# microsoft/ANCE

Hardware: NVIDIA H100
Metric: ANN-refresh throughput: passages encoded/sec + queries top-200/sec, 8.8M x 768 (higher is better)
Workload: dtype fp16

## Files before the change

### ance_b200/csrc/capi.cu

```cuda
#include <atomic>
#include <mutex>
#include <string.h>
#include <vector>

#include "common.h"
#include "gemm_store.cuh"

namespace ance {

static thread_local char g_err[1024] = "";
std::atomic<int64_t> g_launches{0};

void set_error(const char* fmt, ...) {
  va_list ap;
  va_start(ap, fmt);
  vsnprintf(g_err, sizeof(g_err), fmt, ap);
  va_end(ap);
}

void count_launch(int n) { g_launches.fetch_add(n, std::memory_order_relaxed); }

static bool g_prof_on = false;
static std::mutex g_prof_mu;
static std::vector<cudaEvent_t> g_ev_pool;
// ... 9 lines not shown
}
void prof_begin(int cls, cudaStream_t st) {
  if (!g_prof_on) return;
  std::lock_guard<std::mutex> lk(g_prof_mu);
  g_open[cls] = get_event();
  cudaEventRecord(g_open[cls], st);
}
void prof_end(int cls, cudaStream_t st) {
  if (!g_prof_on) return;
  std::lock_guard<std::mutex> lk(g_prof_mu);
  cudaEvent_t b = get_event();
  cudaEventRecord(b, st);
  g_spans[cls].push_back({g_open[cls], b});
}

}

extern "C" const char* ance_version(void) { return "ance_b200 0.1 (sm_90a)"; }
extern "C" const char* ance_last_error(void) { return ance::g_err; }
extern "C" int64_t ance_launch_count(void) { return ance::g_launches.load(); }

extern "C" int ance_profile_enable(int on) {
  std::lock_guard<std::mutex> lk(ance::g_prof_mu);
  ance::g_prof_on = on != 0;
  return ANCE_OK;
}

extern "C" int ance_profile_read(double* ms_by_class, int64_t* launches_by_class, int n, int reset) {
  ANCE_REQUIRE(ms_by_class && launches_by_class && n > 0 && n <= ance::kNumCls, "ance_profile_read: bad arguments");
  ANCE_CUDA(cudaDeviceSynchronize());
  std::lock_guard<std::mutex> lk(ance::g_prof_mu);
  for (int c = 0; c < ance::kNumCls; ++c) {
    for (auto& s : ance::g_spans[c]) {
      float ms = 0.f;
      if (cudaEventElapsedTime(&ms, s.a, s.b) == cudaSuccess) { ance::g_ms[c] += ms; ance::g_cnt[c] += 1; }
      ance::g_ev_pool.push_back(s.a);
      ance::g_ev_pool.push_back(s.b);
    }
    ance::g_spans[c].clear();
  }
  for (int c = 0; c < n; ++c) { ms_by_class[c] = ance::g_ms[c]; launches_by_class[c] = ance::g_cnt[c]; }
  if (reset) for (int c = 0; c < ance::kNumCls; ++c) { ance::g_ms[c] = 0; ance::g_cnt[c] = 0; }
  return ANCE_OK;
}

namespace {

template <int BN, int STAGES, int CG, uint32_t FMT>
int run_dbg(const void* A, const void* B, int M, int N, int K, const float* bias, const void* R, int act, void* C,
            float* C32, cudaStream_t st) {
  constexpr int EW = 4;
  using Ep = gemm::EpStore<BN, EW>;
  CUtensorMap tmA, tmB;
  if (!tc05_host::make_tmap_2d_16b(&tmA, A, M, K, K, gemm::BM) ||
      !tc05_host::make_tmap_2d_16b(&tmB, B, N, K, K, BN / CG)) {
    ance::set_error("cuTensorMapEncodeTiled failed (M=%d N=%d K=%d)", M, N, K);
    return ANCE_ERR_CUDA;
  }
  gemm::WorkShape ws = gemm::make_shape(M, N, K, BN, CG, 0);
  typename Ep::Params p;
  memset(&p, 0, sizeof(p));
  if (C && !gemm::make_store_tmap(&p.tmC, C, M, N, N)) {
    ance::set_error("cuTensorMapEncodeTiled failed for the output (M=%d N=%d)", M, N);
    return ANCE_ERR_CUDA;
  }
  if (C && R && !gemm::make_store_tmap(&p.tmR, const_cast<void*>(R), M, N, N)) {
    ance::set_error("cuTensorMapEncodeTiled failed for the residual (M=%d N=%d)", M, N);
    return ANCE_ERR_CUDA;
  }
  p.C = reinterpret_cast<uint16_t*>(C);
  p.C32 = C32;
  p.bias = bias;
  p.R = reinterpret_cast<const uint16_t*>(R);
  p.ldc = N;
  p.ldc32 = N;
  p.ldr = N;
  p.act = act;
  ANCE_CUDA((gemm::launch<Ep, BN, STAGES, CG, EW, FMT>(tmA, tmB, ws, p, 0, st)));
  ance::count_launch(1);
  return ANCE_OK;
}

template <uint32_t FMT>
int dispatch_dbg(int variant, const void* A, const void* B, int M, int N, int K, const float* bias, const void* R,
                 int act, void* C, float* C32, cudaStream_t st) {
  switch (variant) {
    case 0: return run_dbg<128, 4, 1, FMT>(A, B, M, N, K, bias, R, act, C, C32, st);
    case 1: return run_dbg<128, 3, 1, FMT>(A, B, M, N, K, bias, R, act, C, C32, st);
    case 2: return run_dbg<128, 4, 2, FMT>(A, B, M, N, K, bias, R, act, C, C32, st);
    case 3: return run_dbg<64, 6, 2, FMT>(A, B, M, N, K, bias, R, act, C, C32, st);
    case 4: return run_dbg<64, 6, 1, FMT>(A, B, M, N, K, bias, R, act, C, C32, st);
    default: ance::set_error("ance_dbg_gemm: unknown variant %d", variant); return ANCE_ERR_INVALID;
  }
}

}

extern "C" int ance_dbg_gemm(const void* A_dev, const void* B_dev, int M, int N, int K, int fmt, int variant,
                             const float* bias_dev, const void* residual_bf16_dev, int act, void* C_bf16_dev,
                             float* C_f32_dev, void* stream) {
  ANCE_REQUIRE(A_dev && B_dev && M > 0 && N > 0 && K > 0, "ance_dbg_gemm: null operand or empty shape");
  ANCE_REQUIRE(K % 8 == 0 && N % 8 == 0, "ance_dbg_gemm: K and N must be multiples of 8 (16-byte rows)");
  cudaStream_t st = reinterpret_cast<cudaStream_t>(stream);
  if (fmt == ANCE_FMT_BF16)
    return dispatch_dbg<tc05::kFmtBF16>(variant, A_dev, B_dev, M, N, K, bias_dev, residual_bf16_dev, act, C_bf16_dev,
                                        C_f32_dev, st);
  if (fmt == ANCE_FMT_FP16)
    return dispatch_dbg<tc05::kFmtF16>(variant, A_dev, B_dev, M, N, K, bias_dev, residual_bf16_dev, act, C_bf16_dev,
                                       C_f32_dev, st);
  ance::set_error("ance_dbg_gemm: unknown operand format %d", fmt);
  return ANCE_ERR_INVALID;
}
```

### ance_b200/csrc/encoder.cu

```cuda
#include <math.h>
#include <stdlib.h>
#include <string.h>

#include <cmath>
#include <map>
#include <vector>

#include "attention.cuh"
#include "attn_bwd_long.cuh"
#include "common.h"
#include "dropout.cuh"
#include "encoder_bwd.cuh"
#include "gemm_store.cuh"

namespace {

constexpr float kLog2e = 1.4426950408889634f;

struct EmbedParams {
  const int32_t* ids;
  const int32_t* lens;
  const uint8_t* mask;
  int B, L, H;
  int roberta;
// ... 375 lines not shown
  float *word = nullptr, *pos = nullptr, *type = nullptr;
  float *eg = nullptr, *eb = nullptr;
  std::vector<LayerDev> layers;
  uint16_t* head_w = nullptr;
  float *head_b = nullptr, *head_g = nullptr, *head_bt = nullptr;
  uint16_t *X = nullptr, *QKV = nullptr, *CTX = nullptr, *T = nullptr, *X1 = nullptr, *FF = nullptr;
  float* kbias = nullptr;
  uint16_t *cls_ctx = nullptr, *cls_x = nullptr;
  int32_t* seq_row0 = nullptr;
  int32_t *row_lo = nullptr, *row_hi = nullptr;
  int2* tile_kv = nullptr;
  float* head_tmp = nullptr;
  int* err_flag = nullptr;
  uint16_t* dbg = nullptr;
  int dbg_tokens = 0;
  float* dbg_grads = nullptr;
  int dbg_grads_tokens = 0;
  bool dbg_grads_valid = false;
  int prune_last_layer = 1;
  int varlen_align = 1;
  std::vector<void*> allocs;
  struct TrainRecord {
    int B, L;
    float p_hidden, p_attn;
    uint64_t seed;
    int n_tiles;
  };
  std::map<const void*, TrainRecord> train_shapes;
  int train_max_len = 128;
  struct LayerT { uint16_t *wqkv, *wo, *w1, *w2; };
  std::vector<LayerT> wt;
  uint16_t* head_wt = nullptr;
  bool wt_stale = true;
  void* bwd_scratch = nullptr;
  std::vector<bwd::RefreshPiece> refresh_table;
  bwd::RefreshPiece* refresh_dev = nullptr;
  size_t refresh_cap = 0;
  size_t bwd_scratch_bytes = 0;
};

namespace {

int require_sm90(int* dev_out) {
  int dev = 0, major = 0, minor = 0;
  ANCE_CUDA(cudaGetDevice(&dev));
  cudaDeviceGetAttribute(&major, cudaDevAttrComputeCapabilityMajor, dev);
  cudaDeviceGetAttribute(&minor, cudaDevAttrComputeCapabilityMinor, dev);
  if (major != 9 || minor != 0) {
    ance::set_error("device %d has compute capability %d.%d; libance_b200 is built for sm_90a only (no CPU fallback)", dev, major, minor);
    return ANCE_ERR_CUDA;
  }
  if (dev_out) *dev_out = dev;
  return ANCE_OK;
}

template <class T>
T* dev_alloc(ance_encoder* e, size_t n) {
  void* p = nullptr;
  if (cudaMalloc(&p, n * sizeof(T)) != cudaSuccess) return nullptr;
  e->allocs.push_back(p);
  return reinterpret_cast<T*>(p);
}

float* upload_f32(ance_encoder* e, const float* h, size_t n) {
  float* d = dev_alloc<float>(e, n);
  if (d) cudaMemcpy(d, h, n * 4, cudaMemcpyHostToDevice);
  return d;
}

uint16_t* upload_16(ance_encoder* e, const float* h, size_t n) {
  std::vector<uint16_t> tmp(n);
  if (e->fmt == tc05::kFmtBF16) for (size_t i = 0; i < n; ++i) tmp[i] = act16::Act<tc05::kFmtBF16>::from_float_host(h[i]);
  else for (size_t i = 0; i < n; ++i) tmp[i] = act16::Act<tc05::kFmtF16>::from_float_host(h[i]);
  uint16_t* d = dev_alloc<uint16_t>(e, n);
  if (d) cudaMemcpy(d, tmp.data(), n * 2, cudaMemcpyHostToDevice);
  return d;
}

int gelu_form() {
  static const int form = getenv("ANCE_B200_GELU") ? atoi(getenv("ANCE_B200_GELU")) : 2;
  return form;
}

template <uint32_t FMT, bool kDrop = false>
int linear(const uint16_t* A, size_t lda, int M, const uint16_t* W, int N, int K, const float* bias,
           const uint16_t* R, int act, uint16_t* C, float* C32, cudaStream_t st, int cls = ance::kClsGemm,
           size_t ldr = 0, const drop::Cfg* dc = nullptr) {
  constexpr int BN = 128, CG = 1, EW = 4, STAGES = 4;
  using Ep = gemm::EpStore<BN, EW, FMT, kDrop>;
  CUtensorMap tmA, tmB;
  if (!tc05_host::make_tmap_2d_16b(&tmA, A, M, K, lda, gemm::BM) || !tc05_host::make_tmap_2d_16b(&tmB, W, N, K, K, BN / CG)) {
    ance::set_error("encoder: cuTensorMapEncodeTiled failed (M=%d N=%d K=%d)", M, N, K);
    return ANCE_ERR_CUDA;
  }
  gemm::WorkShape ws = gemm::make_shape(M, N, K, BN, CG, 0);
  typename Ep::Params p;
  memset(&p, 0, sizeof(p));
  if (C && !gemm::make_store_tmap(&p.tmC, C, M, N, N)) {
    ance::set_error("encoder: cuTensorMapEncodeTiled failed for the output (M=%d N=%d)", M, N);
    return ANCE_ERR_CUDA;
  }
  if (ldr == 0) ldr = N;
  if (C && R && !gemm::make_store_tmap(&p.tmR, const_cast<uint16_t*>(R), M, N, static_cast<int>(ldr))) {
    ance::set_error("encoder: cuTensorMapEncodeTiled failed for the residual (M=%d N=%d)", M, N);
    return ANCE_ERR_CUDA;
  }
  p.C = C;
  p.C32 = C32;
  p.bias = bias;
  p.R = R;
  p.ldc = N;
  p.ldc32 = N;
  p.ldr = static_cast<int>(ldr);
  p.act = act;
  if constexpr (kDrop) p.drop = *dc;
  {
    ance::ProfScope ps(cls, st);
    ANCE_CUDA((gemm::launch<Ep, BN, STAGES, CG, EW, FMT>(tmA, tmB, ws, p, 0, st)));
  }
  ance::count_launch(1);
  return ANCE_OK;
}

int g_ln_rows_per_warp = 2;

template <uint32_t FMT>
int layer_norm(const void* in, bool in_f32, size_t in_ld, int rows, int H, const float* g, const float* b, float eps,
               uint16_t* out16, float* out32, cudaStream_t st) {
  const int blocks = (rows + 7) / 8;
  const int nv = H / 256;
  ance::ProfScope ps(ance::kClsNorm, st);
  if (!in_f32 && out16 && !out32 && nv == 3 && g_ln_rows_per_warp > 1 && rows >= 4096) {
    const uint16_t* src = reinterpret_cast<const uint16_t*>(in);
    if (g_ln_rows_per_warp == 2) ln_rows_multi_kernel<3, 2, FMT><<<(rows + 15) / 16, 256, 0, st>>>(src, in_ld, rows, H, g, b, eps, out16);
    else if (g_ln_rows_per_warp == 3) ln_rows_packed_kernel<3, 2, FMT><<<(rows + 15) / 16, 256, 0, st>>>(src, in_ld, rows, H, g, b, eps, out16);
    else ln_rows_multi_kernel<3, 4, FMT><<<(rows + 31) / 32, 256, 0, st>>>(src, in_ld, rows, H, g, b, eps, out16);
    ANCE_CUDA(cudaGetLastError());
    ance::count_launch(1);
    return ANCE_OK;
  }
#define LN_CASE(NV_)                                                                                            \
  if (in_f32) ln_rows_kernel<NV_, true, FMT><<<blocks, 256, 0, st>>>(in, in_ld, rows, H, g, b, eps, out16, out32); \
  else ln_rows_kernel<NV_, false, FMT><<<blocks, 256, 0, st>>>(in, in_ld, rows, H, g, b, eps, out16, out32)
  if (nv == 3) { LN_CASE(3); }
  else if (nv == 4) { LN_CASE(4); }
  else if (nv == 1) { LN_CASE(1); }
  else if (nv == 2) { LN_CASE(2); }
  else { ance::set_error("encoder: hidden size %d unsupported", H); return ANCE_ERR_UNSUPPORTED; }
#undef LN_CASE
  ANCE_CUDA(cudaGetLastError());
  ance::count_launch(1);
  return ANCE_OK;
}

template <uint32_t FMT>
int set_attention_attrs() {
  ANCE_CUDA(cudaFuncSetAttribute(attn::attention_multi_kernel<false, FMT>, cudaFuncAttributeMaxDynamicSharedMemorySize, attn::Smem::kDynamic));
  ANCE_CUDA(cudaFuncSetAttribute(attn::attention_single_kernel<false, FMT>, cudaFuncAttributeMaxDynamicSharedMemorySize, attn::SmemSingle::kDynamic));
  ANCE_CUDA(cudaFuncSetAttribute(attn::attention_single_kernel<true, FMT>, cudaFuncAttributeMaxDynamicSharedMemorySize, attn::SmemSingle::kDynamic));
  ANCE_CUDA(cudaFuncSetAttribute(attn::attention_multi_kernel<true, FMT>, cudaFuncAttributeMaxDynamicSharedMemorySize, attn::Smem::kDynamic));
  ANCE_CUDA(cudaFuncSetAttribute(attn::attention_single_kernel<false, FMT, true>, cudaFuncAttributeMaxDynamicSharedMemorySize, attn::SmemSingle::kDynamic));
  ANCE_CUDA(cudaFuncSetAttribute(attn::attention_single_kernel<true, FMT, true>, cudaFuncAttributeMaxDynamicSharedMemorySize, attn::SmemSingle::kDynamic));
  ANCE_CUDA(cudaFuncSetAttribute(attn::attention_multi_kernel<false, FMT, true>, cudaFuncAttributeMaxDynamicSharedMemorySize, attn::Smem::kDynamic));
  ANCE_CUDA(cudaFuncSetAttribute(attn::attention_multi_kernel<true, FMT, true>, cudaFuncAttributeMaxDynamicSharedMemorySize, attn::Smem::kDynamic));
  return ANCE_OK;
}

struct AttentionLaunch {
  CUtensorMap tmQKV, tmCTX;
  attn::Params ap;
  int grid;
  bool packed, single;
};

int make_attention(AttentionLaunch& a, const uint16_t* qkv, uint16_t* ctx, int n_tokens, int L, int heads,
                   const float* kbias, const int32_t* row_lo, const int32_t* row_hi, const int2* tile_kv) {
  const int H = heads * attn::kDh;
  if (!tc05_host::make_tmap_2d_16b(&a.tmQKV, qkv, n_tokens, 3 * H, 3 * H, attn::kTile)) {
    ance::set_error("encoder: cuTensorMapEncodeTiled failed for QKV");
    return ANCE_ERR_CUDA;
  }
  if (!tc05_host::make_tmap_2d_16b(&a.tmCTX, ctx, n_tokens, H, H, attn::kTile)) {
    ance::set_error("encoder: cuTensorMapEncodeTiled failed for the attention output");
    return ANCE_ERR_CUDA;
  }
// ... 1561 lines not shown
```

### ance_b200/csrc/gemm_core.cuh

```cuda
#pragma once
#include "tc05.cuh"

namespace gemm {

using namespace tc05;

constexpr int BM = 128;
constexpr int BK = 64;
constexpr int MMA_K = 16;

struct WorkShape {
  int M, N, K;
  int num_m_blks;
  int num_n_blks;
  int n_splits;
  int n_blks_per_split;
  unsigned long long hint_a, hint_b;
  int* pace;
  int pace_window;
  int pace_stride;
};

static __device__ __noinline__ void pace_wait(int* pace, int window, int me, int n_clusters, int stride, int seq) {
  volatile int* vp = pace;
// ... 110 lines not shown
  } else if (warp >= 4 && warp < 8) {
    Ring<STAGES> ring;
    uint32_t acc_phase = 0;
    auto release = [&](int stage) {
      __syncwarp();
      if (lane == 0) {
        mbar_arrive(&empty_bar[stage]);
        if constexpr (CG == 2) mbar_arrive_cluster(&empty_bar[stage], cta_rank ^ 1u);
      }
    };
    for (int w = cluster_id; w < total_work; w += num_clusters) {
      const int m_blk = w / ws.n_splits, split = w - m_blk * ws.n_splits;
      const int nb0 = split * ws.n_blks_per_split;
      const int nb1 = min(nb0 + ws.n_blks_per_split, ws.num_n_blks);
      (void)m_blk;
      for (int nb = nb0; nb < nb1; ++nb) {
        float acc0[BN / 2], acc1[BN / 2];
#pragma unroll
        for (int i = 0; i < BN / 2; ++i) acc0[i] = acc1[i] = 0.f;
        int prev_stage = -1;
        for (int kb = 0; kb < num_kb; ++kb) {
          mbar_wait(&full_bar[ring.stage], ring.phase, 3);
          const uint32_t sa = smem_u32(smem + ring.stage * Plan::kStageBytes);
          const uint32_t sb = sa + Plan::kABytes;
          wgmma_fence();
#pragma unroll
          for (int k = 0; k < BK / MMA_K; ++k) {
            const uint64_t bdesc = make_desc_k_sw128(sb + k * MMA_K * 2);
            wgmma_tile<FMT, BN>(acc0, make_desc_k_sw128(sa + k * MMA_K * 2), bdesc, 1u);
            wgmma_tile<FMT, BN>(acc1, make_desc_k_sw128(sa + 64 * 128 + k * MMA_K * 2), bdesc, 1u);
          }
          wgmma_commit();
          wgmma_wait<1>();
          wgmma_fence_regs(acc0);
          wgmma_fence_regs(acc1);
          if (prev_stage >= 0) release(prev_stage);
          prev_stage = ring.stage;
          ring.advance();
        }
        wgmma_wait<0>();
        wgmma_fence_regs(acc0);
        wgmma_fence_regs(acc1);
        if (prev_stage >= 0) release(prev_stage);
        mbar_wait(aempty_bar, acc_phase ^ 1, 2);
        acc_store_frag(acc_tile, Plan::kAccPitch, 0, 0, acc0);
        acc_store_frag(acc_tile, Plan::kAccPitch, 64, 0, acc1);
        __syncwarp();
        if (lane == 0) mbar_arrive(afull_bar);
        acc_phase ^= 1;
      }
    }
  } else if (warp >= 8) {
    Ep epi;
    EpiCtx cx;
    cx.quad = warp & 3;
    cx.epi_warp = warp - 8;
    cx.lane = lane;
    cx.work_seq = 0;
    cx.ep_smem = smem + Plan::kEpOffset;
    uint32_t acc_phase = 0;
    const uint32_t tacc = smem_u32(acc_tile) / 4u + static_cast<uint32_t>((cx.quad * 32 + lane) * Plan::kAccPitch);
    for (int w = cluster_id; w < total_work; w += num_clusters, ++cx.work_seq) {
      cx.m_blk = w / ws.n_splits;
      cx.split = w - cx.m_blk * ws.n_splits;
      cx.nb0 = cx.split * ws.n_blks_per_split;
      cx.nb1 = min(cx.nb0 + ws.n_blks_per_split, ws.num_n_blks);
      cx.row0 = (cx.m_blk * CG + (int)cta_rank) * BM;
      epi.begin_work(ep, ws, cx);
      for (int nb = cx.nb0; nb < cx.nb1; ++nb) {
        mbar_wait(afull_bar, acc_phase, 4);
        epi.tile(ep, ws, cx, tacc, nb);
        __syncwarp();
        if (lane == 0) mbar_arrive(aempty_bar);
        acc_phase ^= 1;
      }
      epi.end_work(ep, ws, cx);
    }
    epi.end_kernel(ep, cx);
  }

  if constexpr (CG == 2) cluster_sync_all();
}

constexpr int kMaxDevices = 64;

inline int current_device() {
  int dev = 0;
  cudaGetDevice(&dev);
  return (dev >= 0 && dev < kMaxDevices) ? dev : 0;
}

inline int sm_count() {
  static int n[kMaxDevices] = {};
  const int dev = current_device();
  if (!n[dev]) cudaDeviceGetAttribute(&n[dev], cudaDevAttrMultiProcessorCount, dev);
  return n[dev];
}

template <class Ep, int BN, int STAGES, int CG, int EPI_WARPS, uint32_t FMT>
cudaError_t launch(const CUtensorMap& tmA, const CUtensorMap& tmB, const WorkShape& ws,
                   const typename Ep::Params& ep, int max_ctas, cudaStream_t stream) {
  using Plan = SmemPlan<BN, STAGES, CG, Ep::kSmemBytes>;
  auto kern = tc05_gemm_kernel<Ep, BN, STAGES, CG, EPI_WARPS, FMT>;
  static bool configured[kMaxDevices] = {};
  const int dev = current_device();
  if (!configured[dev]) {
    cudaError_t e = cudaFuncSetAttribute(kern, cudaFuncAttributeMaxDynamicSharedMemorySize, Plan::kDynamicBytes);
    if (e != cudaSuccess) return e;
    configured[dev] = true;
  }
  const int total = ws.num_m_blks * ws.n_splits;
  int clusters = min(total, (max_ctas > 0 ? max_ctas : sm_count()) / CG);
  if (clusters < 1) clusters = 1;
  cudaLaunchConfig_t cfg = {};
  cfg.gridDim = dim3(clusters * CG);
  cfg.blockDim = dim3(256 + 32 * EPI_WARPS);
  cfg.dynamicSmemBytes = Plan::kDynamicBytes;
  cfg.stream = stream;
  cudaLaunchAttribute attr[1];
  attr[0].id = cudaLaunchAttributeClusterDimension;
  attr[0].val.clusterDim.x = CG;
  attr[0].val.clusterDim.y = 1;
  attr[0].val.clusterDim.z = 1;
  cfg.attrs = attr;
  cfg.numAttrs = 1;
  return cudaLaunchKernelEx(&cfg, kern, tmA, tmB, ws, ep);
}

inline WorkShape make_shape(int M, int N, int K, int BN, int CG, int n_splits ) {
  WorkShape ws;
  ws.M = M;
  ws.N = N;
  ws.K = K;
  ws.num_m_blks = (M + BM * CG - 1) / (BM * CG);
  ws.num_n_blks = (N + BN - 1) / BN;
  if (n_splits <= 0 || n_splits > ws.num_n_blks) n_splits = ws.num_n_blks;
  ws.n_blks_per_split = (ws.num_n_blks + n_splits - 1) / n_splits;
  ws.n_splits = (ws.num_n_blks + ws.n_blks_per_split - 1) / ws.n_blks_per_split;
  ws.hint_a = ws.hint_b = 0;
  ws.pace = nullptr;
  ws.pace_window = 0;
  ws.pace_stride = 1;
  return ws;
}

}
```

### ance_b200/csrc/gemm_store.cuh

```cuda
#pragma once
#include "act16.cuh"
#include "dropout.cuh"
#include "gemm_core.cuh"

namespace gemm {

__device__ __forceinline__ float rcp_approx(float x) {
  float r;
  asm("rcp.approx.ftz.f32 %0, %1;" : "=f"(r) : "f"(x));
  return r;
}
__device__ __forceinline__ float ex2_approx(float x) {
  float r;
  asm("ex2.approx.ftz.f32 %0, %1;" : "=f"(r) : "f"(x));
  return r;
}

__device__ __forceinline__ uint64_t pack2(float a, float b) {
  uint64_t r;
  asm("mov.b64 %0, {%1, %2};" : "=l"(r) : "f"(a), "f"(b));
  return r;
}
__device__ __forceinline__ void unpack2(uint64_t v, float& a, float& b) {
  asm("mov.b64 {%0, %1}, %2;" : "=f"(a), "=f"(b) : "l"(v));
// ... 157 lines not shown
      if (col0 >= ws.N) break;
      const bool tma_res = (p.R != nullptr) && (p.C != nullptr) && (p.C32 == nullptr);
      uint64_t* rbar = reinterpret_cast<uint64_t*>(cx.ep_smem + kColGroups * kSlabBytes) + cgi;
      uint8_t* rowp = slab + r_in_tile * 128;
      if (tma_res && issuer) {
        tc05::bulk_wait_read_all();
        tc05::mbar_arrive_expect_tx(rbar, kSlabBytes);
        tc05::tma_load_2d(slab, &p.tmR, rbar, col0, cx.row0, tc05::kEvictFirst);
      }
      constexpr bool kLean = EPI_WARPS > 8;
      uint32_t va[32], vb[kLean ? 1 : 32];
      tc05::acc_ld_x32(tacc + col_in_tile, va);
      if constexpr (!kLean) tc05::acc_ld_x32(tacc + col_in_tile + 32, vb);
      if (!tma_res && p.C) {
        if (issuer) tc05::bulk_wait_read_all();
        tc05::named_bar_sync(2 + cgi, 128);
      }
#pragma unroll
      for (int h = 0; h < 2; ++h) {
        float f[32];
        if constexpr (kLean) {
          if (h == 1) {
            tc05::acc_ld_x32(tacc + col_in_tile + 32, va);
          }
#pragma unroll
          for (int i = 0; i < 32; ++i) f[i] = __uint_as_float(va[i]);
        } else {
#pragma unroll
          for (int i = 0; i < 32; ++i) f[i] = __uint_as_float(h == 0 ? va[i] : vb[i]);
        }
        finish_chunk(p, ws, f, row, row_ok, col0 + h * 32, !tma_res);
        if (p.C32 && row_ok) {
          float* o = p.C32 + (size_t)row * p.ldc32 + col0 + h * 32;
          if (col0 + h * 32 + 32 <= ws.N) {
#pragma unroll
            for (int j = 0; j < 8; ++j)
              reinterpret_cast<float4*>(o)[j] = make_float4(f[j * 4], f[j * 4 + 1], f[j * 4 + 2], f[j * 4 + 3]);
          } else {
            for (int i = 0; i < 32; ++i)
              if (col0 + h * 32 + i < ws.N) o[i] = f[i];
          }
        }
        if (p.C) {
          if (tma_res && h == 0) tc05::mbar_wait(rbar, rphase, 20);
#pragma unroll
          for (int q = 0; q < 4; ++q) {
            uint4* cp = reinterpret_cast<uint4*>(rowp + (((h * 4 + q) ^ (r_in_tile & 7)) * 16));
            if (tma_res) {
              const uint4 rv = *cp;
              const uint32_t rh[4] = {rv.x, rv.y, rv.z, rv.w};
#pragma unroll
              for (int t = 0; t < 4; ++t) {
                const float2 x = A16::unpack2(rh[t]);
                f[q * 8 + t * 2] += x.x;
                f[q * 8 + t * 2 + 1] += x.y;
              }
            }
            uint4 o;
            o.x = A16::pack2(f[q * 8 + 0], f[q * 8 + 1]);
            o.y = A16::pack2(f[q * 8 + 2], f[q * 8 + 3]);
            o.z = A16::pack2(f[q * 8 + 4], f[q * 8 + 5]);
            o.w = A16::pack2(f[q * 8 + 6], f[q * 8 + 7]);
            *cp = o;
          }
        }
      }
      if (p.C) {
        if (tma_res) rphase ^= 1;
        tc05::fence_proxy_async_smem();
        tc05::named_bar_sync(2 + cgi, 128);
        if (issuer) {
          tc05::tma_store_2d(&p.tmC, slab, col0, cx.row0);
          tc05::bulk_commit_group();
        }
      }
    }
  }
};

inline bool make_store_tmap(CUtensorMap* tm, void* C, int M, int N, int ldc) {
  return tc05_host::make_tmap_2d_16b(tm, C, M, N, ldc, BM, 64);
}

}
```

### ance_b200/csrc/tc05.cuh

```cuda
#pragma once

#include <cuda.h>
#include <cuda_bf16.h>
#include <cuda_fp16.h>
#include <cuda_runtime.h>
#include <stdint.h>
#include <stdio.h>

namespace tc05 {

__device__ __forceinline__ uint32_t smem_u32(const void* p) {
  return static_cast<uint32_t>(__cvta_generic_to_shared(p));
}

__device__ __forceinline__ uint32_t cluster_ctarank() {
  uint32_t r;
  asm volatile("mov.u32 %0, %%cluster_ctarank;" : "=r"(r));
  return r;
}

__device__ __forceinline__ void cluster_sync_all() {
  asm volatile("barrier.cluster.arrive.release.aligned;\n" ::: "memory");
  asm volatile("barrier.cluster.wait.acquire.aligned;\n" ::: "memory");
}
// ... 16 lines not shown

__device__ __forceinline__ void mbar_arrive_expect_tx(uint64_t* bar, uint32_t bytes) {
  asm volatile("mbarrier.arrive.expect_tx.shared::cta.b64 _, [%0], %1;" ::"r"(smem_u32(bar)), "r"(bytes)
               : "memory");
}

__device__ __forceinline__ void mbar_arrive(uint64_t* bar) {
  asm volatile("mbarrier.arrive.shared::cta.b64 _, [%0];" ::"r"(smem_u32(bar)) : "memory");
}

__device__ __forceinline__ void mbar_arrive_cluster(uint64_t* bar, uint32_t cta) {
  uint32_t remote;
  asm volatile("mapa.shared::cluster.u32 %0, %1, %2;" : "=r"(remote) : "r"(smem_u32(bar)), "r"(cta));
  asm volatile("mbarrier.arrive.shared::cluster.b64 _, [%0];" ::"r"(remote) : "memory");
}

__device__ __forceinline__ uint32_t mbar_try_wait(uint64_t* bar, uint32_t parity) {
  uint32_t ok;
  asm volatile(
      "{\n\t"
      ".reg .pred p;\n\t"
      "mbarrier.try_wait.parity.shared::cta.b64 p, [%1], %2;\n\t"
      "selp.u32 %0, 1, 0, p;\n\t"
      "}"
      : "=r"(ok)
      : "r"(smem_u32(bar)), "r"(parity)
      : "memory");
  return ok;
}

#ifndef TC05_WATCHDOG_CYCLES
#define TC05_WATCHDOG_CYCLES 8000000000ll
#endif
__device__ __forceinline__ void mbar_wait(uint64_t* bar, uint32_t parity, int tag = 0) {
  (void)tag;
  if (mbar_try_wait(bar, parity)) return;
  long long t0 = clock64();
  uint32_t spins = 0;
  while (!mbar_try_wait(bar, parity)) {
    if ((++spins & 0x3FFu) == 0 && clock64() - t0 > TC05_WATCHDOG_CYCLES) asm volatile("trap;");
  }
}

__device__ __forceinline__ void tma_prefetch_desc(const CUtensorMap* tm) {
  asm volatile("prefetch.tensormap [%0];" ::"l"(reinterpret_cast<uint64_t>(tm)) : "memory");
}

__device__ __forceinline__ void tma_load_2d(void* smem_dst, const CUtensorMap* tm, uint64_t* bar, int c0,
                                            int c1, uint64_t hint) {
  asm volatile(
      "cp.async.bulk.tensor.2d.shared::cluster.global.mbarrier::complete_tx::bytes.L2::cache_hint"
      " [%0], [%1, {%3, %4}], [%2], %5;"
      :
      : "r"(smem_u32(smem_dst)), "l"(reinterpret_cast<uint64_t>(tm)), "r"(smem_u32(bar)), "r"(c0), "r"(c1),
        "l"(hint)
      : "memory");
}

__device__ __forceinline__ void tma_load_2d_multicast(void* smem_dst, const CUtensorMap* tm, uint64_t* bar, int c0,
                                                      int c1, uint16_t cta_mask, uint64_t hint) {
  asm volatile(
      "cp.async.bulk.tensor.2d.shared::cluster.global.mbarrier::complete_tx::bytes.multicast::cluster.L2::cache_hint"
      " [%0], [%1, {%3, %4}], [%2], %5, %6;"
      :
      : "r"(smem_u32(smem_dst)), "l"(reinterpret_cast<uint64_t>(tm)), "r"(smem_u32(bar)), "r"(c0), "r"(c1),
        "h"(cta_mask), "l"(hint)
      : "memory");
}

__device__ __forceinline__ void tma_store_2d(const CUtensorMap* tm, const void* smem_src, int c0, int c1) {
  asm volatile("cp.async.bulk.tensor.2d.global.shared::cta.bulk_group [%0, {%2, %3}], [%1];"
               :
               : "l"(reinterpret_cast<uint64_t>(tm)), "r"(smem_u32(smem_src)), "r"(c0), "r"(c1)
               : "memory");
}
__device__ __forceinline__ void bulk_commit_group() { asm volatile("cp.async.bulk.commit_group;" ::: "memory"); }
__device__ __forceinline__ void bulk_wait_read_all() { asm volatile("cp.async.bulk.wait_group.read 0;" ::: "memory"); }
__device__ __forceinline__ void bulk_wait_all() { asm volatile("cp.async.bulk.wait_group 0;" ::: "memory"); }

__device__ __forceinline__ void named_bar_sync(int id, int threads) {
  asm volatile("bar.sync %0, %1;" ::"r"(id), "r"(threads) : "memory");
}

__device__ __forceinline__ uint64_t make_desc_k_sw128(uint32_t smem_addr) {
  uint64_t d = 0;
  d |= static_cast<uint64_t>((smem_addr & 0x3FFFFu) >> 4);
  d |= static_cast<uint64_t>(1) << 16;
  d |= static_cast<uint64_t>(1024 >> 4) << 32;
  d |= static_cast<uint64_t>(1) << 62;
  return d;
}

__device__ __forceinline__ uint64_t make_desc_mn_sw128(uint32_t smem_addr, uint32_t lbo_bytes,
                                                       uint32_t sbo_bytes) {
  uint64_t d = 0;
  d |= static_cast<uint64_t>((smem_addr & 0x3FFFFu) >> 4);
  d |= static_cast<uint64_t>((lbo_bytes >> 4) & 0x3FFFu) << 16;
  d |= static_cast<uint64_t>((sbo_bytes >> 4) & 0x3FFFu) << 32;
  d |= static_cast<uint64_t>(1) << 62;
  return d;
}

enum : uint32_t { kFmtF16 = 0, kFmtBF16 = 1 };

__device__ __forceinline__ void wgmma_fence() { asm volatile("wgmma.fence.sync.aligned;" ::: "memory"); }
__device__ __forceinline__ void wgmma_commit() { asm volatile("wgmma.commit_group.sync.aligned;" ::: "memory"); }
template <int N>
__device__ __forceinline__ void wgmma_wait() { asm volatile("wgmma.wait_group.sync.aligned %0;" ::"n"(N) : "memory"); }
template <int R>
__device__ __forceinline__ void wgmma_fence_regs(float (&d)[R]) {
#pragma unroll
  for (int i = 0; i < R; ++i) asm volatile("" : "+f"(d[i])::"memory");
}

#define TC05_R8(i) "+f"(d[i]), "+f"(d[i + 1]), "+f"(d[i + 2]), "+f"(d[i + 3]), "+f"(d[i + 4]), "+f"(d[i + 5]), "+f"(d[i + 6]), "+f"(d[i + 7])
#define TC05_R32 TC05_R8(0), TC05_R8(8), TC05_R8(16), TC05_R8(24)
#define TC05_R64 TC05_R32, TC05_R8(32), TC05_R8(40), TC05_R8(48), TC05_R8(56)
#define TC05_S32                                                                  \
  "%0, %1, %2, %3, %4, %5, %6, %7, %8, %9, %10, %11, %12, %13, %14, %15, "        \
  "%16, %17, %18, %19, %20, %21, %22, %23, %24, %25, %26, %27, %28, %29, %30, %31"
#define TC05_S64                                                                  \
  TC05_S32 ", "                                                                   \
  "%32, %33, %34, %35, %36, %37, %38, %39, %40, %41, %42, %43, %44, %45, %46, %47, " \
  "%48, %49, %50, %51, %52, %53, %54, %55, %56, %57, %58, %59, %60, %61, %62, %63"
#define TC05_WGMMA(NAME, INSTR, NR, SLIST, RLIST, IA, IB, IP, IT)                                                     \
  template <int kTransB>                                                                                              \
  __device__ __forceinline__ void NAME(float (&d)[NR], uint64_t adesc, uint64_t bdesc, uint32_t accumulate) {        \
    asm volatile("{\n\t.reg .pred p;\n\tsetp.ne.b32 p, %" IP ", 0;\n\t" INSTR " {" SLIST "}, %" IA ", %" IB           \
                 ", p, 1, 1, 0, %" IT ";\n\t}"                                                                        \
                 : RLIST                                                                                              \
                 : "l"(adesc), "l"(bdesc), "r"(accumulate), "n"(kTransB));                                            \
  }
TC05_WGMMA(wgmma_m64n128k16_bf16, "wgmma.mma_async.sync.aligned.m64n128k16.f32.bf16.bf16", 64, TC05_S64, TC05_R64, "64", "65", "66", "67")
TC05_WGMMA(wgmma_m64n128k16_f16, "wgmma.mma_async.sync.aligned.m64n128k16.f32.f16.f16", 64, TC05_S64, TC05_R64, "64", "65", "66", "67")
TC05_WGMMA(wgmma_m64n64k16_bf16, "wgmma.mma_async.sync.aligned.m64n64k16.f32.bf16.bf16", 32, TC05_S32, TC05_R32, "32", "33", "34", "35")
TC05_WGMMA(wgmma_m64n64k16_f16, "wgmma.mma_async.sync.aligned.m64n64k16.f32.f16.f16", 32, TC05_S32, TC05_R32, "32", "33", "34", "35")

template <uint32_t FMT, int kTransB>
__device__ __forceinline__ void wgmma_n128(float (&d)[64], uint64_t adesc, uint64_t bdesc, uint32_t accumulate) {
  if constexpr (FMT == kFmtBF16) wgmma_m64n128k16_bf16<kTransB>(d, adesc, bdesc, accumulate);
  else wgmma_m64n128k16_f16<kTransB>(d, adesc, bdesc, accumulate);
}
template <uint32_t FMT, int kTransB>
__device__ __forceinline__ void wgmma_n64(float (&d)[32], uint64_t adesc, uint64_t bdesc, uint32_t accumulate) {
  if constexpr (FMT == kFmtBF16) wgmma_m64n64k16_bf16<kTransB>(d, adesc, bdesc, accumulate);
  else wgmma_m64n64k16_f16<kTransB>(d, adesc, bdesc, accumulate);
}

#define TC05_WGMMA_RS(NAME, INSTR)                                                                                    \
  __device__ __forceinline__ void NAME(float (&d)[32], const uint32_t (&a)[4], uint64_t bdesc) {                     \
    asm volatile("{\n\t.reg .pred p;\n\tsetp.ne.b32 p, %37, 0;\n\t" INSTR " {" TC05_S32                              \
                 "}, {%32, %33, %34, %35}, %36, p, 1, 1, 1;\n\t}"                                                     \
                 : TC05_R32                                                                                           \
                 : "r"(a[0]), "r"(a[1]), "r"(a[2]), "r"(a[3]), "l"(bdesc), "r"(1u));                                  \
  }
TC05_WGMMA_RS(wgmma_m64n64k16_rs_bf16, "wgmma.mma_async.sync.aligned.m64n64k16.f32.bf16.bf16")
TC05_WGMMA_RS(wgmma_m64n64k16_rs_f16, "wgmma.mma_async.sync.aligned.m64n64k16.f32.f16.f16")
template <uint32_t FMT>
__device__ __forceinline__ void wgmma_n64_rs(float (&d)[32], const uint32_t (&a)[4], uint64_t bdesc) {
  if constexpr (FMT == kFmtBF16) wgmma_m64n64k16_rs_bf16(d, a, bdesc);
  else wgmma_m64n64k16_rs_f16(d, a, bdesc);
}
template <int R>
__device__ __forceinline__ void wgmma_fence_regs(uint32_t (&a)[R]) {
#pragma unroll
  for (int i = 0; i < R; ++i) asm volatile("" : "+r"(a[i])::"memory");
}


template <int R>
__device__ __forceinline__ void acc_store_frag(float* tile, int pitch, int r0, int c0, const float (&d)[R]) {
  const int t = threadIdx.x & 127;
  const int r = r0 + 16 * (t >> 5) + ((t & 31) >> 2);
  const int c = c0 + 2 * (t & 3);
#pragma unroll
  for (int j = 0; j < R / 4; ++j) {
    *reinterpret_cast<float2*>(tile + r * pitch + c + 8 * j) = make_float2(d[4 * j], d[4 * j + 1]);
    *reinterpret_cast<float2*>(tile + (r + 8) * pitch + c + 8 * j) = make_float2(d[4 * j + 2], d[4 * j + 3]);
  }
}

__device__ __forceinline__ void acc_ld_x32(uint32_t waddr, uint32_t* v) {
#pragma unroll
  for (int i = 0; i < 32; i += 4)
    asm volatile("ld.shared.v4.u32 {%0, %1, %2, %3}, [%4];"
                 : "=r"(v[i]), "=r"(v[i + 1]), "=r"(v[i + 2]), "=r"(v[i + 3])
                 : "r"((waddr + i) * 4u)
                 : "memory");
}

template <int kStages>
struct Ring {
  uint32_t stage = 0, phase = 0;
  __device__ __forceinline__ void advance() {
    if (++stage == kStages) {
      stage = 0;
      phase ^= 1;
    }
  }
};

}

namespace tc05_host {

typedef CUresult (*EncodeTiledFn)(CUtensorMap*, CUtensorMapDataType, cuuint32_t, void*, const cuuint64_t*,
                                  const cuuint64_t*, const cuuint32_t*, const cuuint32_t*, CUtensorMapInterleave,
                                  CUtensorMapSwizzle, CUtensorMapL2promotion, CUtensorMapFloatOOBfill);

inline EncodeTiledFn encode_fn() {
  static EncodeTiledFn fn = nullptr;
  if (!fn) {
    void* p = nullptr;
    cudaDriverEntryPointQueryResult q;
    if (cudaGetDriverEntryPoint("cuTensorMapEncodeTiled", &p, cudaEnableDefault, &q) != cudaSuccess ||
        q != cudaDriverEntryPointSuccess)
      return nullptr;
    fn = reinterpret_cast<EncodeTiledFn>(p);
  }
  return fn;
// ... 18 lines not shown
```

Measured before the change: 18760.

## Add warp-specialized 128x256 GEMM with register reallocation for large linears

Adds a persistent GEMM kernel with 128x256 tiles. It uses a TMA producer warp and two dedicated epilogue-store warps in the first warpgroup, and two consumer warpgroups issuing m64n256 wgmma, with setmaxnreg shifting registers to the consumers. The encoder's linear layer now routes to this kernel when there is no activation, no dropout, a 16-bit output and at least ten waves of tiles. The wider tile is meant to raise operand reuse and tensor-core efficiency on the big projection GEMMs, at the cost of fewer pipeline stages (3) and higher register pressure.

```diff
diff --git a/ance_b200/csrc/capi.cu b/ance_b200/csrc/capi.cu
--- a/ance_b200/csrc/capi.cu
+++ b/ance_b200/csrc/capi.cu
@@ -115,6 +115,33 @@
 }
 
 template <uint32_t FMT>
+int run_dbg_wide(const void* A, const void* B, int M, int N, int K, const float* bias, const void* R, int act, void* C,
+                 float* C32, cudaStream_t st) {
+  using Ep = gemm::EpStoreWide<>;
+  ANCE_REQUIRE(C && !C32, "ance_dbg_gemm: variant 5 writes a 16-bit output only");
+  CUtensorMap tmA, tmB;
+  if (!tc05_host::make_tmap_2d_16b(&tmA, A, M, K, K, gemm::BM) ||
+      !tc05_host::make_tmap_2d_16b(&tmB, B, N, K, K, gemm::kWideBN)) {
+    ance::set_error("cuTensorMapEncodeTiled failed (M=%d N=%d K=%d)", M, N, K);
+    return ANCE_ERR_CUDA;
+  }
+  gemm::WorkShape ws = gemm::make_shape(M, N, K, gemm::kWideBN, 1, 0);
+  typename Ep::Params p;
+  memset(&p, 0, sizeof(p));
+  if (!gemm::make_store_wide_tmap(&p.tmC, C, M, N, N) ||
+      (R && !gemm::make_store_wide_tmap(&p.tmR, const_cast<void*>(R), M, N, N))) {
+    ance::set_error("cuTensorMapEncodeTiled failed for the output or residual (M=%d N=%d)", M, N);
+    return ANCE_ERR_CUDA;
+  }
+  p.bias = bias;
+  p.R = reinterpret_cast<const uint16_t*>(R);
+  p.act = act;
+  ANCE_CUDA((gemm::launch_wide<Ep, FMT>(tmA, tmB, ws, p, 0, st)));
+  ance::count_launch(1);
+  return ANCE_OK;
+}
+
+template <uint32_t FMT>
 int dispatch_dbg(int variant, const void* A, const void* B, int M, int N, int K, const float* bias, const void* R,
                  int act, void* C, float* C32, cudaStream_t st) {
   switch (variant) {
@@ -123,6 +150,7 @@
     case 2: return run_dbg<128, 4, 2, FMT>(A, B, M, N, K, bias, R, act, C, C32, st);
     case 3: return run_dbg<64, 6, 2, FMT>(A, B, M, N, K, bias, R, act, C, C32, st);
     case 4: return run_dbg<64, 6, 1, FMT>(A, B, M, N, K, bias, R, act, C, C32, st);
+    case 5: return run_dbg_wide<FMT>(A, B, M, N, K, bias, R, act, C, C32, st);
     default: ance::set_error("ance_dbg_gemm: unknown variant %d", variant); return ANCE_ERR_INVALID;
   }
 }
diff --git a/ance_b200/csrc/encoder.cu b/ance_b200/csrc/encoder.cu
--- a/ance_b200/csrc/encoder.cu
+++ b/ance_b200/csrc/encoder.cu
@@ -481,10 +481,44 @@
   return form;
 }
 
+template <uint32_t FMT>
+int linear_wide(const uint16_t* A, size_t lda, int M, const uint16_t* W, int N, int K, const float* bias,
+                const uint16_t* R, uint16_t* C, cudaStream_t st, int cls, size_t ldr) {
+  using Ep = gemm::EpStoreWide<FMT>;
+  CUtensorMap tmA, tmB;
+  if (!tc05_host::make_tmap_2d_16b(&tmA, A, M, K, lda, gemm::BM) ||
+      !tc05_host::make_tmap_2d_16b(&tmB, W, N, K, K, gemm::kWideBN)) {
+    ance::set_error("encoder: cuTensorMapEncodeTiled failed (M=%d N=%d K=%d)", M, N, K);
+    return ANCE_ERR_CUDA;
+  }
+  const gemm::WorkShape ws = gemm::make_shape(M, N, K, gemm::kWideBN, 1, 0);
+  typename Ep::Params p;
+  memset(&p, 0, sizeof(p));
+  if (!gemm::make_store_wide_tmap(&p.tmC, C, M, N, N) ||
+      (R && !gemm::make_store_wide_tmap(&p.tmR, const_cast<uint16_t*>(R), M, N, static_cast<int>(ldr)))) {
+    ance::set_error("encoder: cuTensorMapEncodeTiled failed for the output or residual (M=%d N=%d)", M, N);
+    return ANCE_ERR_CUDA;
+  }
+  p.bias = bias;
+  p.R = R;
+  {
+    ance::ProfScope ps(cls, st);
+    ANCE_CUDA((gemm::launch_wide<Ep, FMT>(tmA, tmB, ws, p, 0, st)));
+  }
+  ance::count_launch(1);
+  return ANCE_OK;
+}
+
+constexpr int kWideMinWaves = 10;
+
 template <uint32_t FMT, bool kDrop = false>
 int linear(const uint16_t* A, size_t lda, int M, const uint16_t* W, int N, int K, const float* bias,
            const uint16_t* R, int act, uint16_t* C, float* C32, cudaStream_t st, int cls = ance::kClsGemm,
            size_t ldr = 0, const drop::Cfg* dc = nullptr) {
+  if (ldr == 0) ldr = N;
+  if (!kDrop && C && !C32 && act == 0 &&
+      (long long)((M + gemm::BM - 1) / gemm::BM) * ((N + gemm::kWideBN - 1) / gemm::kWideBN) >= (long long)kWideMinWaves * gemm::sm_count())
+    return linear_wide<FMT>(A, lda, M, W, N, K, bias, R, C, st, cls, ldr);
   constexpr int BN = 128, CG = 1, EW = 4, STAGES = 4;
   using Ep = gemm::EpStore<BN, EW, FMT, kDrop>;
   CUtensorMap tmA, tmB;
@@ -499,7 +533,6 @@
     ance::set_error("encoder: cuTensorMapEncodeTiled failed for the output (M=%d N=%d)", M, N);
     return ANCE_ERR_CUDA;
   }
-  if (ldr == 0) ldr = N;
   if (C && R && !gemm::make_store_tmap(&p.tmR, const_cast<uint16_t*>(R), M, N, static_cast<int>(ldr))) {
     ance::set_error("encoder: cuTensorMapEncodeTiled failed for the residual (M=%d N=%d)", M, N);
     return ANCE_ERR_CUDA;
diff --git a/ance_b200/csrc/gemm_core.cuh b/ance_b200/csrc/gemm_core.cuh
--- a/ance_b200/csrc/gemm_core.cuh
+++ b/ance_b200/csrc/gemm_core.cuh
@@ -216,6 +216,130 @@
   if constexpr (CG == 2) cluster_sync_all();
 }
 
+constexpr int kWideBN = 256;
+constexpr int kWideStages = 3;
+
+template <int EP_SMEM>
+struct WideSmemPlan {
+  static constexpr int kABytes = BM * BK * 2;
+  static constexpr int kBBytes = kWideBN * BK * 2;
+  static constexpr int kStageBytes = kABytes + kBBytes;
+  static constexpr int kRingBytes = kWideStages * kStageBytes;
+  static constexpr int kEpOffset = kRingBytes;
+  static constexpr int kBarOffset = kEpOffset + EP_SMEM;
+  static constexpr int kBarBytes = (2 * kWideStages + 4) * 8;
+  static constexpr int kTotal = kBarOffset + kBarBytes;
+  static constexpr int kDynamicBytes = kTotal + 1024;
+  static_assert(kDynamicBytes <= 232448, "GEMM shared memory exceeds 227 KB");
+};
+
+template <class Ep, uint32_t FMT>
+__global__ void __launch_bounds__(384, 1)
+tc05_gemm_wide_kernel(const __grid_constant__ CUtensorMap tmA, const __grid_constant__ CUtensorMap tmB,
+                      const WorkShape ws, const __grid_constant__ typename Ep::Params ep) {
+  using Plan = WideSmemPlan<Ep::kSmemBytes>;
+  extern __shared__ uint8_t smem_raw[];
+  uint8_t* smem = reinterpret_cast<uint8_t*>((reinterpret_cast<uintptr_t>(smem_raw) + 1023) & ~uintptr_t(1023));
+  uint64_t* full_bar = reinterpret_cast<uint64_t*>(smem + Plan::kBarOffset);
+  uint64_t* empty_bar = full_bar + kWideStages;
+  uint64_t* ready_bar = empty_bar + kWideStages;
+  uint64_t* out_bar = ready_bar + 2;
+
+  const int warp = threadIdx.x >> 5;
+  const int lane = threadIdx.x & 31;
+  const int wg = warp >> 2;
+  const int total_work = ws.num_m_blks * ws.num_n_blks;
+  const int num_kb = (ws.K + BK - 1) / BK;
+
+  if (threadIdx.x == 0) {
+    tma_prefetch_desc(&tmA);
+    tma_prefetch_desc(&tmB);
+    for (int s = 0; s < kWideStages; ++s) {
+      mbar_init(&full_bar[s], 1);
+      mbar_init(&empty_bar[s], 8);
+    }
+    for (int g = 0; g < 2; ++g) {
+      mbar_init(&ready_bar[g], 1);
+      mbar_init(&out_bar[g], 4);
+    }
+    fence_barrier_init();
+  }
+  __syncthreads();
+
+  if (wg == 0) {
+    setmaxnreg_dec<40>();
+    if (warp == 0 && lane == 0) {
+      Ring<kWideStages> ring;
+      for (int w = blockIdx.x; w < total_work; w += gridDim.x) {
+        const int m_blk = w / ws.num_n_blks, nb = w - m_blk * ws.num_n_blks;
+        for (int kb = 0; kb < num_kb; ++kb) {
+          mbar_wait(&empty_bar[ring.stage], ring.phase ^ 1, 1);
+          uint8_t* sa = smem + ring.stage * Plan::kStageBytes;
+          mbar_arrive_expect_tx(&full_bar[ring.stage], Plan::kStageBytes);
+          tma_load_2d(sa, &tmA, &full_bar[ring.stage], kb * BK, m_blk * BM, Ep::kHintA);
+          tma_load_2d(sa + Plan::kABytes, &tmB, &full_bar[ring.stage], kb * BK, nb * kWideBN, Ep::kHintB);
+          ring.advance();
+        }
+      }
+    } else if ((warp == 1 || warp == 2) && lane == 0) {
+      const int g = warp - 1;
+      uint8_t* half = smem + Plan::kEpOffset + g * (Ep::kSmemBytes / 2);
+      uint32_t phase = 0;
+      for (int w = blockIdx.x; w < total_work; w += gridDim.x) {
+        const int m_blk = w / ws.num_n_blks, nb = w - m_blk * ws.num_n_blks;
+        const int row0 = m_blk * BM + 64 * g, col0 = nb * kWideBN;
+        Ep::fill(ep, ws, half, &ready_bar[g], row0, col0);
+        mbar_wait(&out_bar[g], phase, 2);
+        phase ^= 1;
+        Ep::drain(ep, ws, half, row0, col0);
+      }
+      bulk_wait_all();
+    }
+  } else {
+    setmaxnreg_inc<232>();
+    const int g = wg - 1;
+    uint8_t* half = smem + Plan::kEpOffset + g * (Ep::kSmemBytes / 2);
+    Ring<kWideStages> ring;
+    uint32_t phase = 0;
+    auto release = [&](int stage) {
+      __syncwarp();
+      if (lane == 0) mbar_arrive(&empty_bar[stage]);
+    };
+    for (int w = blockIdx.x; w < total_work; w += gridDim.x) {
+      const int m_blk = w / ws.num_n_blks, nb = w - m_blk * ws.num_n_blks;
+      float acc[128];
+#pragma unroll
+      for (int i = 0; i < 128; ++i) acc[i] = 0.f;
+      int prev_stage = -1;
+      for (int kb = 0; kb < num_kb; ++kb) {
+        mbar_wait(&full_bar[ring.stage], ring.phase, 3);
+        const uint32_t sa = smem_u32(smem + ring.stage * Plan::kStageBytes);
+        const uint32_t sb = sa + Plan::kABytes;
+        wgmma_fence();
+#pragma unroll
+        for (int k = 0; k < BK / MMA_K; ++k)
+          wgmma_n256<FMT, 0>(acc, make_desc_k_sw128(sa + g * 64 * 128 + k * MMA_K * 2),
+                             make_desc_k_sw128(sb + k * MMA_K * 2), 1u);
+        wgmma_commit();
+        wgmma_wait<1>();
+        wgmma_fence_regs(acc);
+        if (prev_stage >= 0) release(prev_stage);
+        prev_stage = ring.stage;
+        ring.advance();
+      }
+      wgmma_wait<0>();
+      wgmma_fence_regs(acc);
+      release(prev_stage);
+      mbar_wait(&ready_bar[g], phase, 4);
+      phase ^= 1;
+      Ep::tile(ep, ws, acc, half, nb * kWideBN);
+      fence_proxy_async_smem();
+      __syncwarp();
+      if (lane == 0) mbar_arrive(&out_bar[g]);
+    }
+  }
+}
+
 constexpr int kMaxDevices = 64;
 
 inline int current_device() {
@@ -261,6 +385,23 @@
   return cudaLaunchKernelEx(&cfg, kern, tmA, tmB, ws, ep);
 }
 
+template <class Ep, uint32_t FMT>
+cudaError_t launch_wide(const CUtensorMap& tmA, const CUtensorMap& tmB, const WorkShape& ws,
+                        const typename Ep::Params& ep, int max_ctas, cudaStream_t stream) {
+  using Plan = WideSmemPlan<Ep::kSmemBytes>;
+  auto kern = tc05_gemm_wide_kernel<Ep, FMT>;
+  static bool configured[kMaxDevices] = {};
+  const int dev = current_device();
+  if (!configured[dev]) {
+    cudaError_t e = cudaFuncSetAttribute(kern, cudaFuncAttributeMaxDynamicSharedMemorySize, Plan::kDynamicBytes);
+    if (e != cudaSuccess) return e;
+    configured[dev] = true;
+  }
+  const int ctas = max(1, min(ws.num_m_blks * ws.num_n_blks, max_ctas > 0 ? max_ctas : sm_count()));
+  kern<<<ctas, 384, Plan::kDynamicBytes, stream>>>(tmA, tmB, ws, ep);
+  return cudaGetLastError();
+}
+
 inline WorkShape make_shape(int M, int N, int K, int BN, int CG, int n_splits ) {
   WorkShape ws;
   ws.M = M;
diff --git a/ance_b200/csrc/gemm_store.cuh b/ance_b200/csrc/gemm_store.cuh
--- a/ance_b200/csrc/gemm_store.cuh
+++ b/ance_b200/csrc/gemm_store.cuh
@@ -263,4 +263,95 @@
   return tc05_host::make_tmap_2d_16b(tm, C, M, N, ldc, BM, 64);
 }
 
-}
+template <uint32_t FMT = tc05::kFmtBF16>
+struct EpStoreWide {
+  using A16 = act16::Act<FMT>;
+  static constexpr uint64_t kHintA = tc05::kEvictNormal;
+  static constexpr uint64_t kHintB = tc05::kEvictLast;
+  static constexpr int kSlabBytes = 64 * 128;
+  static constexpr int kSmemBytes = 2 * 4 * kSlabBytes;
+
+  struct alignas(64) Params {
+    CUtensorMap tmC;
+    CUtensorMap tmR;
+    const float* bias;
+    const uint16_t* R;
+    int act;
+  };
+
+  __device__ static int slabs(const WorkShape& ws, int row0, int col0) {
+    return row0 < ws.M ? min(4, (ws.N - col0 + 63) / 64) : 0;
+  }
+
+  __device__ static void fill(const Params& p, const WorkShape& ws, uint8_t* half, uint64_t* bar, int row0, int col0) {
+    const int n = p.R ? slabs(ws, row0, col0) : 0;
+    if (n == 0) {
+      tc05::mbar_arrive(bar);
+      return;
+    }
+    tc05::mbar_arrive_expect_tx(bar, n * kSlabBytes);
+    for (int s = 0; s < n; ++s) tc05::tma_load_2d(half + s * kSlabBytes, &p.tmR, bar, col0 + 64 * s, row0, tc05::kEvictFirst);
+  }
+
+  __device__ static void drain(const Params& p, const WorkShape& ws, uint8_t* half, int row0, int col0) {
+    const int n = slabs(ws, row0, col0);
+    for (int s = 0; s < n; ++s) tc05::tma_store_2d(&p.tmC, half + s * kSlabBytes, col0 + 64 * s, row0);
+    tc05::bulk_commit_group();
+    tc05::bulk_wait_read_all();
+  }
+
+  template <int ACT>
+  __device__ __forceinline__ static void slab(const Params& p, const WorkShape& ws, const float* acc, uint8_t* sl,
+                                              int col, int r, int c) {
+    uint32_t* w0[8];
+    float2 b[8];
+    uint32_t x0[8], x1[8];
+#pragma unroll
+    for (int i = 0; i < 8; ++i) {
+      w0[i] = reinterpret_cast<uint32_t*>(sl + r * 128 + ((i ^ (r & 7)) << 4) + 2 * c);
+      b[i] = (p.bias && col + 8 * i < ws.N) ? __ldg(reinterpret_cast<const float2*>(p.bias + col + 8 * i))
+                                            : make_float2(0.f, 0.f);
+      x0[i] = p.R ? *w0[i] : 0u;
+      x1[i] = p.R ? *(w0[i] + 8 * 128 / 4) : 0u;
+    }
+#pragma unroll
+    for (int i = 0; i < 8; ++i) {
+      float v0 = acc[4 * i], v1 = acc[4 * i + 1], v2 = acc[4 * i + 2], v3 = acc[4 * i + 3];
+      if (p.bias) {
+        v0 += b[i].x; v1 += b[i].y; v2 += b[i].x; v3 += b[i].y;
+      }
+      if constexpr (ACT == 1) {
+        gelu_erf2(v0, v1);
+        gelu_erf2(v2, v3);
+      } else if constexpr (ACT == 2) {
+        gelu_logistic2(v0, v1);
+        gelu_logistic2(v2, v3);
+      }
+      if (p.R) {
+        const float2 y0 = A16::unpack2(x0[i]), y1 = A16::unpack2(x1[i]);
+        v0 += y0.x; v1 += y0.y; v2 += y1.x; v3 += y1.y;
+      }
+      *w0[i] = A16::pack2(v0, v1);
+      *(w0[i] + 8 * 128 / 4) = A16::pack2(v2, v3);
+    }
+  }
+
+  __device__ static void tile(const Params& p, const WorkShape& ws, const float (&acc)[128], uint8_t* half, int col0) {
+    const int t = threadIdx.x & 127;
+    const int r = 16 * (t >> 5) + ((t & 31) >> 2);
+    const int c = 2 * (t & 3);
+#pragma unroll
+    for (int s = 0; s < 4; ++s) {
+      const int col = col0 + 64 * s + c;
+      if (p.act == 1) slab<1>(p, ws, acc + 32 * s, half + s * kSlabBytes, col, r, c);
+      else if (p.act == 2) slab<2>(p, ws, acc + 32 * s, half + s * kSlabBytes, col, r, c);
+      else slab<0>(p, ws, acc + 32 * s, half + s * kSlabBytes, col, r, c);
+    }
+  }
+};
+
+inline bool make_store_wide_tmap(CUtensorMap* tm, void* C, int M, int N, int ld) {
+  return tc05_host::make_tmap_2d_16b(tm, C, M, N, ld, 64, 64);
+}
+
+}
diff --git a/ance_b200/csrc/tc05.cuh b/ance_b200/csrc/tc05.cuh
--- a/ance_b200/csrc/tc05.cuh
+++ b/ance_b200/csrc/tc05.cuh
@@ -122,6 +122,11 @@
   asm volatile("bar.sync %0, %1;" ::"r"(id), "r"(threads) : "memory");
 }
 
+template <int N>
+__device__ __forceinline__ void setmaxnreg_dec() { asm volatile("setmaxnreg.dec.sync.aligned.u32 %0;" ::"n"(N)); }
+template <int N>
+__device__ __forceinline__ void setmaxnreg_inc() { asm volatile("setmaxnreg.inc.sync.aligned.u32 %0;" ::"n"(N)); }
+
 __device__ __forceinline__ uint64_t make_desc_k_sw128(uint32_t smem_addr) {
   uint64_t d = 0;
   d |= static_cast<uint64_t>((smem_addr & 0x3FFFFu) >> 4);
@@ -163,6 +168,13 @@
   TC05_S32 ", "                                                                   \
   "%32, %33, %34, %35, %36, %37, %38, %39, %40, %41, %42, %43, %44, %45, %46, %47, " \
   "%48, %49, %50, %51, %52, %53, %54, %55, %56, %57, %58, %59, %60, %61, %62, %63"
+#define TC05_R128 TC05_R64, TC05_R8(64), TC05_R8(72), TC05_R8(80), TC05_R8(88), TC05_R8(96), TC05_R8(104), TC05_R8(112), TC05_R8(120)
+#define TC05_S128                                                                               \
+  TC05_S64 ", "                                                                                 \
+  "%64, %65, %66, %67, %68, %69, %70, %71, %72, %73, %74, %75, %76, %77, %78, %79, "            \
+  "%80, %81, %82, %83, %84, %85, %86, %87, %88, %89, %90, %91, %92, %93, %94, %95, "            \
+  "%96, %97, %98, %99, %100, %101, %102, %103, %104, %105, %106, %107, %108, %109, %110, %111, " \
+  "%112, %113, %114, %115, %116, %117, %118, %119, %120, %121, %122, %123, %124, %125, %126, %127"
 #define TC05_WGMMA(NAME, INSTR, NR, SLIST, RLIST, IA, IB, IP, IT)                                                     \
   template <int kTransB>                                                                                              \
   __device__ __forceinline__ void NAME(float (&d)[NR], uint64_t adesc, uint64_t bdesc, uint32_t accumulate) {        \
@@ -171,11 +183,18 @@
                  : RLIST                                                                                              \
                  : "l"(adesc), "l"(bdesc), "r"(accumulate), "n"(kTransB));                                            \
   }
-TC05_WGMMA(wgmma_m64n128k16_bf16, "wgmma.mma_async.sync.aligned.m64n128k16.f32.bf16.bf16", 64, TC05_S64, TC05_R64, "64", "65", "66", "67")
+TC05_WGMMA(wgmma_m64n256k16_bf16, "wgmma.mma_async.sync.aligned.m64n256k16.f32.bf16.bf16", 128, TC05_S128, TC05_R128, "128", "129", "130", "131")
+TC05_WGMMA(wgmma_m64n256k16_f16, "wgmma.mma_async.sync.aligned.m64n256k16.f32.f16.f16", 128, TC05_S128, TC05_R128, "128", "129", "130", "131")
+TC05_WGMMA(wgmma_m64n128k16_bf16,"wgmma.mma_async.sync.aligned.m64n128k16.f32.bf16.bf16", 64, TC05_S64, TC05_R64, "64", "65", "66", "67")
 TC05_WGMMA(wgmma_m64n128k16_f16, "wgmma.mma_async.sync.aligned.m64n128k16.f32.f16.f16", 64, TC05_S64, TC05_R64, "64", "65", "66", "67")
 TC05_WGMMA(wgmma_m64n64k16_bf16, "wgmma.mma_async.sync.aligned.m64n64k16.f32.bf16.bf16", 32, TC05_S32, TC05_R32, "32", "33", "34", "35")
 TC05_WGMMA(wgmma_m64n64k16_f16, "wgmma.mma_async.sync.aligned.m64n64k16.f32.f16.f16", 32, TC05_S32, TC05_R32, "32", "33", "34", "35")
 
+template <uint32_t FMT, int kTransB>
+__device__ __forceinline__ void wgmma_n256(float (&d)[128], uint64_t adesc, uint64_t bdesc, uint32_t accumulate) {
+  if constexpr (FMT == kFmtBF16) wgmma_m64n256k16_bf16<kTransB>(d, adesc, bdesc, accumulate);
+  else wgmma_m64n256k16_f16<kTransB>(d, adesc, bdesc, accumulate);
+}
 template <uint32_t FMT, int kTransB>
 __device__ __forceinline__ void wgmma_n128(float (&d)[64], uint64_t adesc, uint64_t bdesc, uint32_t accumulate) {
   if constexpr (FMT == kFmtBF16) wgmma_m64n128k16_bf16<kTransB>(d, adesc, bdesc, accumulate);
```

Measured after the change: 19870, median of 6. +5.9%, better.
